# louiskirsch/speechT

Measured on AMD Instinct MI355X. Metric: utterances/sec (training step, 10 s@16 kHz, batch 32), higher is better.
Workload: dtype f32

## Files before the change

include/speecht_hip.h:

```cpp
#ifndef SPEECHT_HIP_H
#define SPEECHT_HIP_H

#include <stddef.h>
#include <stdint.h>

#ifdef __cplusplus
extern "C" {
#endif

#define ST_OK 0
#define ST_EINVAL (-1)
#define ST_ELAUNCH (-2)
#define ST_EWORKSPACE (-3)
#define ST_ECOMM (-4)

typedef struct st_tensor3 {
  float* base;
  int32_t batch;
  int32_t frames;
  int32_t channels;
  int32_t halo;
  int32_t t_pitch;
  int32_t c_pitch;
} st_tensor3;
// ... 21 lines not shown
size_t st_conv1d_fwd_ws(const st_tensor3* x, const st_tensor3* y, int width);
int st_conv1d_nwc_fwd_ws_f32(const st_tensor3* x, const float* packed, const float* bias, int width,
                             int stride, int pad_left, int relu, const st_tensor3* y, void* workspace,
                             size_t workspace_bytes, void* stream);

int st_conv1d_fft_plan(int width, int frames, int batch, int* n, int* valid, int* blocks, int* bins, int* rows_pad);
int st_gemm_nn_batched_f32(const float* a, int64_t lda, int64_t a_batch, const float* b, int64_t b_batch, float* c,
                           int64_t ldc, int64_t c_batch, int m, int k, int n, int batches, void* stream);
size_t st_gemm_nn_batched_ws_bytes(void);
size_t st_gemm_nn_batched_ctrl_bytes(void);
int st_streamk_lost_ptr(void** device_word);
int st_streamk_lost_count(unsigned* count);
int st_streamk_lost_fetch_async(unsigned* host_word, void* stream);
int st_gemm_nn_batched_ws_f32(const float* a, int64_t lda, int64_t a_batch, const float* b, int64_t b_batch, float* c,
                              int64_t ldc, int64_t c_batch, int m, int k, int n, int batches, void* workspace,
                              size_t workspace_bytes, void* stream);
int st_gemm_nn_batched_bt_ws_f32(const float* a, int64_t lda, int64_t a_batch, const float* bt, int64_t bt_batch, float* c,
                                 int64_t ldc, int64_t c_batch, int m, int k, int n, int batches, void* workspace,
                                 size_t workspace_bytes, void* stream);
int st_gemm_tn_batched_f32(const float* a, int64_t lda, int64_t a_batch, const float* z, int64_t ldz, int64_t z_batch,
                           float* out, int64_t out_batch, int m, int k, int n, int batches, void* stream);
int st_gemm_tn_batched_shared_f32(const float* a, int64_t lda, int64_t a_batch, const float* z, int64_t ldz, int64_t z_batch,
                                  float* out, int64_t out_batch, int m, int k, int n, int batches, int z_batch_shift, void* stream);
int st_gemm_nn_g3_batched_f32(const float* a, int64_t lda, int64_t a_batch, const int64_t* a_off, const float* b, int64_t ldb,
                              int64_t b_batch, const int64_t* b_off, int b_transposed, float* c, int64_t ldc, int64_t c_batch,
                              int64_t c_off2, int m, int k, int n, int batches, void* stream);
int st_gemm_tn_g3_batched_f32(const float* a, int64_t lda, int64_t a_batch, const int64_t* a_off, const float* z, int64_t ldz,
                              int64_t z_batch, const int64_t* z_off, float* out, int64_t out_batch, int64_t out_part, int m, int k,
                              int n, int batches, void* stream);
int st_conv1d_fft_three_products(int width, int cin_pitch, int cout);
size_t st_conv1d_fft_table_floats(void);
int st_conv1d_fft_tables_f32(int width, int pad_left, float* tables, size_t table_floats, void* stream);
size_t st_conv1d_fft_filter_floats(int width, int cin_pitch, int cout);
int st_conv1d_fft_filters_f32(const float* packed, int width, int cin, int cout, int cin_pitch, const float* tables, float* gfwd,
                              void* stream);
size_t st_conv1d_fft_sf_floats(const st_tensor3* x, const st_tensor3* y, int width);
size_t st_conv1d_fft_zf_floats(const st_tensor3* dz, int width);
size_t st_conv1d_fft_ws(const st_tensor3* x, const st_tensor3* y, int width);
int st_conv1d_nwc_fwd_fft_f32(const st_tensor3* x, const float* gfwd, const float* bias, int width, int pad_left, int relu,
                              const st_tensor3* y, const float* tables, float* sf, void* workspace,
                              size_t workspace_bytes, void* stream);
int st_conv1d_nwc_fwd_fft_chain_f32(const st_tensor3* x, const float* gfwd, const float* bias, int width, int pad_left, int relu,
                                    const st_tensor3* y, const float* tables, float* sf, int sf_ready, const float* next_tables,
                                    float* next_sf, int next_width, int next_pad_left, int* next_sf_written, void* workspace,
                                    size_t workspace_bytes, void* stream);
int st_conv1d_fft_dz_spectra_f32(const st_tensor3* dz, int width, const float* tables, float* zf, void* stream);
// ... 257 lines not shown
```

speecht_amd/_lib.py:

```python
import ctypes
import os
from ctypes import POINTER, c_char_p, c_float, c_int, c_int32, c_int64, c_long, c_size_t, c_void_p

from .build import LIB_PATH


class Tensor3(ctypes.Structure):
  _fields_ = [('base', c_void_p), ('batch', c_int32), ('frames', c_int32), ('channels', c_int32),
              ('halo', c_int32), ('t_pitch', c_int32), ('c_pitch', c_int32)]


class SpeechtHipError(RuntimeError):
  pass


_T3P = POINTER(Tensor3)
_SIGNATURES = {
    'st_version': (c_int, []),
    'st_last_error': (c_char_p, []),
    'st_trace_begin': (c_int, []),
    'st_trace_begin_timed': (c_int, []),
    'st_trace_timed_filter': (c_int, [c_char_p]),
    'st_trace_end': (c_size_t, [c_char_p, c_size_t]),
    'st_set_tuning': (c_int, [c_char_p, c_int]),
# ... 3 lines not shown
    'st_unpack_filters_f32': (c_int, [c_void_p, c_int, c_int, c_int, c_int, c_void_p, c_void_p]),
    'st_filters_flip_transpose_f32': (c_int, [c_void_p, c_int, c_int, c_int, c_int, c_int, c_void_p, c_void_p]),
    'st_conv1d_nwc_fwd_f32': (c_int, [_T3P, c_void_p, c_void_p, c_int, c_int, c_int, c_int, _T3P, c_void_p]),
    'st_conv1d_fwd_ws': (c_size_t, [_T3P, _T3P, c_int]),
    'st_conv1d_nwc_fwd_ws_f32': (c_int, [_T3P, c_void_p, c_void_p, c_int, c_int, c_int, c_int, _T3P, c_void_p, c_size_t,
                                          c_void_p]),
    'st_conv1d_fft_plan': (c_int, [c_int, c_int, c_int, POINTER(c_int), POINTER(c_int), POINTER(c_int), POINTER(c_int),
                                   POINTER(c_int)]),
    'st_gemm_nn_batched_f32': (c_int, [c_void_p, c_int64, c_int64, c_void_p, c_int64, c_void_p, c_int64, c_int64, c_int, c_int,
                                       c_int, c_int, c_void_p]),
    'st_gemm_nn_batched_ws_bytes': (c_size_t, []),
    'st_gemm_nn_batched_ctrl_bytes': (c_size_t, []),
    'st_streamk_lost_ptr': (c_int, [POINTER(c_void_p)]),
    'st_streamk_lost_count': (c_int, [POINTER(ctypes.c_uint32)]),
    'st_streamk_lost_fetch_async': (c_int, [c_void_p, c_void_p]),
    'st_gemm_nn_batched_ws_f32': (c_int, [c_void_p, c_int64, c_int64, c_void_p, c_int64, c_void_p, c_int64, c_int64, c_int, c_int,
                                          c_int, c_int, c_void_p, c_size_t, c_void_p]),
    'st_gemm_nn_batched_bt_ws_f32': (c_int, [c_void_p, c_int64, c_int64, c_void_p, c_int64, c_void_p, c_int64, c_int64, c_int, c_int,
                                             c_int, c_int, c_void_p, c_size_t, c_void_p]),
    'st_gemm_tn_batched_f32': (c_int, [c_void_p, c_int64, c_int64, c_void_p, c_int64, c_int64, c_void_p, c_int64, c_int, c_int,
                                       c_int, c_int, c_void_p]),
    'st_gemm_tn_batched_shared_f32': (c_int, [c_void_p, c_int64, c_int64, c_void_p, c_int64, c_int64, c_void_p, c_int64, c_int, c_int,
                                              c_int, c_int, c_int, c_void_p]),
    'st_gemm_nn_g3_batched_f32': (c_int, [c_void_p, c_int64, c_int64, POINTER(c_int64), c_void_p, c_int64, c_int64, POINTER(c_int64), c_int,
                                          c_void_p, c_int64, c_int64, c_int64, c_int, c_int, c_int, c_int, c_void_p]),
    'st_gemm_tn_g3_batched_f32': (c_int, [c_void_p, c_int64, c_int64, POINTER(c_int64), c_void_p, c_int64, c_int64, POINTER(c_int64),
                                          c_void_p, c_int64, c_int64, c_int, c_int, c_int, c_int, c_void_p]),
    'st_conv1d_fft_three_products': (c_int, [c_int, c_int, c_int]),
    'st_conv1d_fft_table_floats': (c_size_t, []),
    'st_conv1d_fft_tables_f32': (c_int, [c_int, c_int, c_void_p, c_size_t, c_void_p]),
    'st_conv1d_fft_filter_floats': (c_size_t, [c_int, c_int, c_int]),
    'st_conv1d_fft_filters_f32': (c_int, [c_void_p, c_int, c_int, c_int, c_int, c_void_p, c_void_p, c_void_p]),
    'st_conv1d_fft_sf_floats': (c_size_t, [_T3P, _T3P, c_int]),
    'st_conv1d_fft_zf_floats': (c_size_t, [_T3P, c_int]),
    'st_conv1d_fft_ws': (c_size_t, [_T3P, _T3P, c_int]),
    'st_conv1d_nwc_fwd_fft_f32': (c_int, [_T3P, c_void_p, c_void_p, c_int, c_int, c_int, _T3P, c_void_p, c_void_p, c_void_p,
                                          c_size_t, c_void_p]),
    'st_conv1d_nwc_fwd_fft_chain_f32': (c_int, [_T3P, c_void_p, c_void_p, c_int, c_int, c_int, _T3P, c_void_p, c_void_p, c_int, c_void_p,
                                                c_void_p, c_int, c_int, POINTER(c_int), c_void_p, c_size_t, c_void_p]),
    'st_conv1d_nwc_bwd_data_fft_chain_f32': (c_int, [_T3P, c_void_p, c_void_p, c_int, c_int, _T3P, _T3P, c_void_p, c_void_p, c_void_p, c_int,
                                                     POINTER(c_int), c_void_p, c_size_t, c_void_p]),
    'st_conv1d_fft_filter_plane_elems': (c_size_t, [c_int, c_int, c_int]),
    'st_conv1d_fft_filters_planes': (c_int, [c_void_p, c_int, c_int, c_int, c_int, c_void_p, c_void_p, c_void_p, c_int, c_void_p]),
    'st_conv1d_fft_planes_ws': (c_size_t, [_T3P, _T3P, c_int, c_int]),
    'st_conv1d_nwc_fwd_fft_planes': (c_int, [_T3P, c_void_p, c_void_p, c_void_p, c_int, c_int, c_int, _T3P, c_void_p, c_void_p, c_void_p,
                                             c_int, c_void_p, c_size_t, c_void_p]),
# ... 225 lines not shown
```

speecht_amd/csrc/conv_fft.hip:

```cpp
#include <algorithm>

#include "st_common.h"

namespace {

typedef float f32x2 __attribute__((ext_vector_type(2)));
typedef float f32x4 __attribute__((ext_vector_type(4)));
typedef float f32x16 __attribute__((ext_vector_type(16)));

constexpr int V = 64;
constexpr int KP = 96;
constexpr int HB = KP / 2;
constexpr int T_FS = 0;
constexpr int T_FZ = T_FS + KP * KP;
constexpr int T_IY = T_FZ + KP * KP;
constexpr int T_IX = T_IY + V * KP;
constexpr int T_TW = T_IX + 3 * V * KP;
constexpr int T_FW = T_TW + 256;
constexpr int T_FP = T_FW + HB * 34 * 2;
constexpr int FUSE_BLOCKS = 8, FUSE_HALO = 4, FUSE_Q = 32 + FUSE_HALO;
constexpr int T_IW = T_FP + FUSE_Q * KP * 2;
constexpr int T_ZP = T_IW + KP * KP;
constexpr int T_END = T_ZP + 32 * KP * 2;
__host__ __device__ inline int fused_column(int q, int hh, int n, int pad_left) {
// ... 456 lines not shown
    for (int i = 0; i < 3; ++i)
#pragma unroll
      for (int r = 0; r < 16; ++r) {
        const int m = i * 32 + (r & 3) + 8 * (r >> 2) + 4 * h;
        const int bin = m < HB ? m : m - HB, col = (m < HB ? 0 : half_next) + c;
        if (bin < bins_next) {
          const long o = (long)bin * bin_stride + (long)row * 2 * half_next;
          out[o + col] = sacc[i][r];
          if (out2) out2[o + (m < HB ? half_next : 0) + c] = m < HB ? -sacc[i][r] : sacc[i][r];
        }
      }
  }
}

template <int HP>
__global__ __launch_bounds__(64 * FUSE_BLOCKS, 1) void idft_ola_dft_rows_kernel(
    const float* __restrict__ in, const float* __restrict__ winv, int blocks, int rows_pad, int bins, int half_in, int nchunks, RowsOut y,
    int pad_left, int right, const float* __restrict__ mask, long mask_batch_stride, int mask_c_pitch,
    const float* __restrict__ wz_below, int bins_below, int half_below, float* __restrict__ zf_below) {
  constexpr int NST = 2 * HP / CH;
  static_assert(2 * HP % CH == 0 && HP <= HB / 2, "pairs per term must fill whole stages");
  __shared__ __attribute__((aligned(16))) float wl[KP * KP];
  __shared__ __attribute__((aligned(16))) float wf[32 * KP * 2];
  __shared__ float spill[FUSE_BLOCKS][2][FUSE_HALO][32];
  const int tid = threadIdx.x, lane = tid & 63, l31 = lane & 31, h = lane >> 5;
  const int wave = __builtin_amdgcn_readfirstlane(tid >> 6);
  const int b = blockIdx.x / nchunks, chunk = blockIdx.x - b * nchunks;
  const int j = wave, row = b * blocks + j, c = chunk * 32 + l31;
  const bool active = j < blocks;
  const long plane = (long)rows_pad * 2 * half_in;
  const bool cok = c < half_in;
  const float* src = in + (long)(active ? row : 0) * 2 * half_in + min(c, half_in - 1);
  auto load = [&](float (&bf)[CH], int st) {
#pragma unroll
    for (int s = 0; s < CH; ++s) {
      const int p = st * CH + s;
      const int bin = (p < HP ? 2 * p : 2 * (p - HP)) + h;
      bf[s] = src[(long)min(bin, bins - 1) * plane + (p < HP ? 0 : half_in)];
    }
  };
  float bfr[NST][CH];
  float mk[2][16];
  if (active) {
#pragma unroll
    for (int st = 0; st < NST; ++st) load(bfr[st], st);
    if (mask) {
      const float* mp = mask + (long)b * mask_batch_stride + min(c, mask_c_pitch - 1);
// ... 13 lines not shown
  f32x16 acc[3];
#pragma unroll
  for (int i = 0; i < 3; ++i)
#pragma unroll
    for (int r = 0; r < 16; ++r) acc[i][r] = 0.f;
  if (active) {
    const float* afrag = wl + 2 * l31 + h;
#pragma unroll
    for (int st = 0; st < NST; ++st) {
      __builtin_amdgcn_sched_barrier(0);
#pragma unroll
      for (int s = 0; s < CH; ++s) {
        const int p = st * CH + s;
        const int bin = (p < HP ? 2 * p : 2 * (p - HP)) + h;
        const unsigned keep = (cok && bin < bins) ? 0xffffffffu : 0u;
        const float v = __uint_as_float(__float_as_uint(bfr[st][s]) & keep);
        const int sidx = p < HP ? p : HB / 2 + (p - HP);
#pragma unroll
        for (int i = 0; i < 3; ++i) acc[i] = __builtin_amdgcn_mfma_f32_32x32x2f32(afrag[(sidx * KP + i * 32) * 2], v, acc[i], 0, 0, 0);
      }
      __builtin_amdgcn_sched_barrier(0);
    }
#pragma unroll
    for (int e = 0; e < FUSE_HALO; ++e) spill[j][h][e][l31] = acc[2][e];
  }
  __syncthreads();
  if (!active) return;
#pragma unroll
  for (int e = 0; e < FUSE_HALO; ++e) {
    if (h == 0) { if (j > 0 && e < right) acc[0][e] += spill[j - 1][1][e][l31]; }
    else { if (j + 1 < blocks && e >= FUSE_HALO - pad_left) acc[1][12 + e] += spill[j + 1][0][e - (FUSE_HALO - pad_left)][l31]; }
  }
#pragma unroll
  for (int i = 0; i < 2; ++i)
#pragma unroll
    for (int r = 0; r < 16; ++r) {
      const int t = j * V + i * 32 + (r & 3) + 8 * (r >> 2) + 4 * h;
      float val = c < y.channels ? acc[i][r] : 0.f;
      if (mask) val = mk[i][r] > 0.f ? val : 0.f;
      val = t < y.frames ? val : 0.f;
      asm volatile("" : "+v"(val));
      acc[i][r] = val;
    }
  if (c < y.c_pitch) {
    float* yp = y.base + (long)b * y.batch_stride + c;
#pragma unroll
    for (int i = 0; i < 2; ++i)
#pragma unroll
      for (int r = 0; r < 16; ++r) {
        const int t = j * V + i * 32 + (r & 3) + 8 * (r >> 2) + 4 * h;
        if (t < y.frames) yp[(long)t * y.c_pitch] = acc[i][r];
      }
  }
  if (!wz_below) return;
// ... 359 lines not shown
int st_gemm_nn_batched_ws_f32(const float* a, int64_t lda, int64_t a_batch, const float* b, int64_t b_batch, float* c, int64_t ldc,
                              int64_t c_batch, int m, int k, int n, int batches, void* workspace, size_t workspace_bytes,
                              void* stream) {
  float* sk = (workspace && workspace_bytes >= st_gemm_nn_batched_ws_bytes()) ? reinterpret_cast<float*>(workspace) : nullptr;
  return st::gemm_nn_batched(a, lda, a_batch, b, b_batch, c, ldc, c_batch, m, k, n, batches, st::as_stream(stream), sk);
}

int st_gemm_nn_batched_bt_ws_f32(const float* a, int64_t lda, int64_t a_batch, const float* bt, int64_t bt_batch, float* c, int64_t ldc,
                                 int64_t c_batch, int m, int k, int n, int batches, void* workspace, size_t workspace_bytes,
                                 void* stream) {
  float* sk = (workspace && workspace_bytes >= st_gemm_nn_batched_ws_bytes()) ? reinterpret_cast<float*>(workspace) : nullptr;
  return st::gemm_nn_batched(a, lda, a_batch, bt, bt_batch, c, ldc, c_batch, m, k, n, batches, st::as_stream(stream), sk, true);
}

int st_gemm_tn_batched_f32(const float* a, int64_t lda, int64_t a_batch, const float* z, int64_t ldz, int64_t z_batch, float* out,
                           int64_t out_batch, int m, int k, int n, int batches, void* stream) {
  return st::gemm_tn_batched(a, lda, a_batch, z, ldz, z_batch, out, out_batch, m, k, n, batches, st::as_stream(stream));
}

int st_gemm_tn_batched_shared_f32(const float* a, int64_t lda, int64_t a_batch, const float* z, int64_t ldz, int64_t z_batch, float* out,
                                  int64_t out_batch, int m, int k, int n, int batches, int z_batch_shift, void* stream) {
  ST_REQUIRE(z_batch_shift >= 0 && z_batch_shift < 8, "gemm_tn_batched_shared: bad shift");
  return st::gemm_tn_batched(a, lda, a_batch, z, ldz, z_batch, out, out_batch, m, k, n, batches, st::as_stream(stream), z_batch_shift);
}

int st_gemm_nn_g3_batched_f32(const float* a, int64_t lda, int64_t a_batch, const int64_t* a_off, const float* b, int64_t ldb, int64_t b_batch,
                              const int64_t* b_off, int b_transposed, float* c, int64_t ldc, int64_t c_batch, int64_t c_off2, int m, int k, int n,
                              int batches, void* stream) {
  ST_REQUIRE(a_off && b_off, "gemm_nn_g3_batched: null offsets");
  const long ao[3] = {(long)a_off[0], (long)a_off[1], (long)a_off[2]}, bo[3] = {(long)b_off[0], (long)b_off[1], (long)b_off[2]};
  return st::gemm_nn_g3_batched(a, lda, a_batch, ao, b, ldb, b_batch, bo, c, ldc, c_batch, c_off2, m, k, n, batches, st::as_stream(stream),
                                b_transposed != 0);
}

int st_gemm_tn_g3_batched_f32(const float* a, int64_t lda, int64_t a_batch, const int64_t* a_off, const float* z, int64_t ldz, int64_t z_batch,
                              const int64_t* z_off, float* out, int64_t out_batch, int64_t out_part, int m, int k, int n, int batches,
                              void* stream) {
  ST_REQUIRE(a_off && z_off, "gemm_tn_g3_batched: null offsets");
  const long ao[3] = {(long)a_off[0], (long)a_off[1], (long)a_off[2]}, zo[3] = {(long)z_off[0], (long)z_off[1], (long)z_off[2]};
  return st::gemm_tn_g3_batched(a, lda, a_batch, ao, z, ldz, z_batch, zo, out, out_batch, out_part, m, k, n, batches, st::as_stream(stream));
}

int st_conv1d_fft_three_products(int width, int cin_pitch, int cout) {
  return g3_form(width, cin_pitch, cout) ? 2 : (zf3_form(width, cout) ? 1 : 0);
}

// ... 398 lines not shown
```

speecht_amd/csrc/conv_gemm.hip:

```cpp
#include <algorithm>
#include <atomic>
#include <cmath>
#include <cstdlib>

#include <type_traits>

#include "st_common.h"
#include "streamk_map.h"

namespace {

typedef float f32x16 __attribute__((ext_vector_type(16)));
typedef float f32x4 __attribute__((ext_vector_type(4)));

constexpr int BK = 32;
constexpr int APITCH = BK + 4;
constexpr int NTHREADS = 256;

struct RowMap {
  int frames;
  int row_stride;
  long batch_stride;
  long row0;
  __device__ __forceinline__ long off(int m) const {
// ... 7 lines not shown
  const float* A;  RowMap amap;
  const float* Bm; int Np;
  float* C;        RowMap cmap;
  const float* mask; RowMap mmap;
  const float* bias;
  int M, Kvalid, Kp, n_store, relu;
  int taps, cp;
  int tiles_m, tiles_n, chunk;
  int gm, tm_per, tn_per;
  int splits, steps_per_split;
  float* slab;
  float* colsum;
  int colsum_rows;
  int batches;
  long a_batch, b_batch, c_batch;
  long bt_ld; int bt_rows;
};


__device__ __forceinline__ void dma16_sv(unsigned lds_byte_addr, const void* sbase, unsigned voff_bytes) {
  unsigned keep;
  asm volatile("s_mov_b32 %0, m0\n\ts_mov_b32 m0, %1\n\ts_nop 0\n\tglobal_load_lds_dwordx4 %2, %3\n\ts_mov_b32 m0, %0"
               : "=&s"(keep) : "s"(lds_byte_addr), "v"(voff_bytes), "s"(sbase) : "memory");
}
__device__ __forceinline__ void dma_wait_all() { asm volatile("s_waitcnt vmcnt(0)" ::: "memory"); }
__device__ __forceinline__ unsigned lds_addr(const float* p) {
  return (unsigned)(size_t)(__attribute__((address_space(3))) const float*)p;
}

template <int N> struct FVec;
template <> struct FVec<1> { typedef float type; };
template <> struct FVec<2> { typedef float type __attribute__((ext_vector_type(2))); };
template <> struct FVec<4> { typedef float type __attribute__((ext_vector_type(4))); };
template <int N> __device__ __forceinline__ float vget(const typename FVec<N>::type& v, int i) { return v[i]; }
template <> __device__ __forceinline__ float vget<1>(const float& v, int) { return v; }
template <int N> __device__ __forceinline__ void vset(typename FVec<N>::type& v, int i, float x) { v[i] = x; }
template <> __device__ __forceinline__ void vset<1>(float& v, int, float x) { v = x; }

__device__ __forceinline__ int swz_slot4(int lane, int row) { return ((lane & 7) ^ ((row >> 1) & 7)) * 4; }
__device__ __forceinline__ int swz_frag(int row, int q, int h) { return row * BK + (((2 * q + h) ^ ((row >> 1) & 7)) * 4); }

template <int BM, int BN, int WMW, int WNW, bool BT>
struct NNStage {
  static constexpr int WTM = BM / WMW, WTN = BN / WNW;
  static constexpr int MT = WTM / 32, NT = WTN / 32;
  static constexpr int A_DMA = BM / 32;
// ... 346 lines not shown
    }
  }
  if (EPI == 1 && p.colsum) {
    bvec out;
#pragma unroll
    for (int n = 0; n < NT; ++n) vset<NT>(out, n, csum[n] + __shfl_xor(csum[n], 32, 64));
    if (h == 0) *reinterpret_cast<bvec*>(p.colsum + (long)(tile_m * WMW + wm) * p.Np + col0) = out;
  }
}

__device__ unsigned g_sk_lost = 0;

struct BinsParams {
  const float* A; const float* B; float* C;
  long lda, ldb, ldc, a_batch, b_batch, c_batch;
  int tiles_m, tiles_n;
  st::SkPlan plan;
  unsigned* ctrl;
  float* partial;
  unsigned epoch;
  unsigned pub_epoch;
};

template <int BM, int BN, int WMW, int WNW, int MINW, bool BT>
__global__ __launch_bounds__(NTHREADS, MINW) void gemm_nn_bins_kernel(BinsParams p) {
  typedef NNStage<BM, BN, WMW, WNW, BT> S;
  constexpr int WTM = S::WTM, WTN = S::WTN, MT = S::MT, NT = S::NT;
  constexpr int A_DMA = S::A_DMA, B_DMA = S::B_DMA, N_DMA = S::N_DMA, A_SZ = S::A_SZ, B_SZ = S::B_SZ;
  constexpr int B_LPR = BN / 4;
  static_assert(WMW * WNW == 4 && MT >= 1 && NT == 2 && A_DMA >= 1 && B_DMA >= 1, "tile config");
  typedef typename FVec<NT>::type bvec;
  typedef unsigned long long u64;

  __shared__ __attribute__((aligned(16))) float smem[2 * A_SZ + 2 * B_SZ + 4];
  float* const As = smem;
  float* const Bs = smem + 2 * A_SZ;
  volatile int* const sk_lost_p = reinterpret_cast<volatile int*>(smem + 2 * A_SZ + 2 * B_SZ);

  const int tid = threadIdx.x;
  const int lane = tid & 63;
  const int wave = __builtin_amdgcn_readfirstlane(tid >> 6);
  const int l31 = lane & 31, h = lane >> 5;
  const int wm = wave / WNW, wn = wave % WNW;
  if (tid == 0) *sk_lost_p = 0;

  const int xcd = blockIdx.x & 7, local = blockIdx.x >> 3;
  const int slot = blockIdx.x;
  st::SkCursor cur;
  if (!st::sk_begin(p.plan, xcd, local, cur)) return;
  const int per_bin = p.tiles_m * p.tiles_n;

  int a_lane[A_DMA];
#pragma unroll
  for (int i = 0; i < A_DMA; ++i) {
    const int row = (wave * A_DMA + i) * 8 + (lane >> 3);
    a_lane[i] = row * (int)p.lda + swz_slot4(lane, row);
  }
  int b_lane[B_DMA];
#pragma unroll
  for (int i = 0; i < B_DMA; ++i) {
    if (BT) {
      const int row = (wave * B_DMA + i) * 8 + (lane >> 3);
      b_lane[i] = row * (int)p.ldb + swz_slot4(lane, row);
    } else {
      b_lane[i] = ((wave * B_DMA + i) * (64 / B_LPR) + lane / B_LPR) * (int)p.ldb + (lane % B_LPR) * 4;
    }
  }
  int bt_frag[4];
  {
    const int row = wn * WTN + l31;
#pragma unroll
    for (int q = 0; q < 4; ++q) bt_frag[q] = swz_frag(row, q, h);
  }
  int a_frag[4];
  {
    const int row = wm * WTM + l31;
#pragma unroll
    for (int q = 0; q < 4; ++q) a_frag[q] = swz_frag(row, q, h);
  }
  const int b_frag = (4 * h) * BN + wn * WTN + NT * l31;
  const int tcol = wn * WTN + NT * l31;

  while (cur.u < cur.u_end) {
    const st::SkPiece pc = st::sk_piece(p.plan, cur);
    cur.u += pc.kt1 - pc.kt0;
    const int bin = pc.tile / per_bin, t = pc.tile - bin * per_bin;
    const int tile_n = t / p.tiles_m, tile_m = t - tile_n * p.tiles_m;
    const int m0 = tile_m * BM, n0 = tile_n * BN;
    const float* __restrict__ Ab = p.A + (long)bin * p.a_batch + (long)m0 * p.lda;
    const float* __restrict__ Bb = p.B + (long)bin * p.b_batch + (BT ? (long)n0 * p.ldb : (long)n0);
    const float* aptr[A_DMA];
    const float* bptr[B_DMA];
#pragma unroll
    for (int i = 0; i < A_DMA; ++i) aptr[i] = Ab + a_lane[i];
#pragma unroll
    for (int i = 0; i < B_DMA; ++i) bptr[i] = Bb + b_lane[i];
    auto dma_piece = [&](int pcx, int k0, int buf) {
      if (pcx < A_DMA) {
        const int i = pcx < A_DMA ? pcx : 0;
        __builtin_amdgcn_global_load_lds((st::gptr_t)(aptr[i] + k0), (st::lptr_t)(As + buf * A_SZ + (wave * A_DMA + i) * 256), 16, 0, 0);
      } else {
        const int i = pcx - A_DMA < B_DMA ? pcx - A_DMA : 0;
        __builtin_amdgcn_global_load_lds((st::gptr_t)(BT ? bptr[i] + k0 : bptr[i] + (long)k0 * p.ldb), (st::lptr_t)(Bs + buf * B_SZ + (wave * B_DMA + i) * 256), 16, 0, 0);
      }
    };

    f32x16 acc[MT][NT] = {};

    int k0 = pc.kt0 * BK;
#pragma unroll
    for (int pcx = 0; pcx < N_DMA; ++pcx) dma_piece(pcx, k0, 0);
    __syncthreads();

    auto stage = [&](auto cur_c, auto more_c) {
      const int nk0 = k0 + BK;
      k0 = nk0;
      S::template run<decltype(cur_c)::value, decltype(more_c)::value>(As, Bs, a_frag, bt_frag, b_frag, acc, 4, dma_piece, nk0);
    };
    const int nk = pc.kt1 - pc.kt0;
    nn_stage_pairs(nk, stage);

    if (pc.kt0 > 0) {
      float* const mine = p.partial + (long)slot * (BM * BN);
#pragma unroll
      for (int i = 0; i < MT; ++i)
#pragma unroll
        for (int r = 0; r < 16; ++r) {
          const int row = wm * WTM + i * 32 + (r & 3) + 8 * (r >> 2) + 4 * h;
          const u64 bits = (u64)__float_as_uint(acc[i][0][r]) | ((u64)__float_as_uint(acc[i][1][r]) << 32);
          __hip_atomic_store(reinterpret_cast<u64*>(mine + row * BN + tcol), bits, __ATOMIC_RELAXED, __HIP_MEMORY_SCOPE_AGENT);
        }
      asm volatile("s_waitcnt vmcnt(0)" ::: "memory");
      __syncthreads();
      if (tid == 0) __hip_atomic_store(p.ctrl + st::SK_FLAGS + slot, p.pub_epoch, __ATOMIC_RELAXED, __HIP_MEMORY_SCOPE_AGENT);
      continue;
    }
    int covered = pc.kt1, src = slot;
    while (covered < p.plan.nk) {
      src += 8;
      if (tid == 0) {
        unsigned* flag = p.ctrl + st::SK_FLAGS + src;
        unsigned spins = 0;
        while (__hip_atomic_load(flag, __ATOMIC_RELAXED, __HIP_MEMORY_SCOPE_AGENT) != p.epoch) {
          __builtin_amdgcn_s_sleep(8);
          if (++spins > (1u << 21)) {
            __hip_atomic_fetch_add(p.ctrl + st::SK_TIMEOUTS, 1u, __ATOMIC_RELAXED, __HIP_MEMORY_SCOPE_AGENT);
            __hip_atomic_fetch_add(&g_sk_lost, 1u, __ATOMIC_RELAXED, __HIP_MEMORY_SCOPE_AGENT);
            *sk_lost_p = 1;
            break;
          }
        }
        __hip_atomic_store(flag, 0u, __ATOMIC_RELAXED, __HIP_MEMORY_SCOPE_AGENT);
      }
      __syncthreads();
      const float poison = *sk_lost_p ? __uint_as_float(0x7fc00000u) : 0.f;
      const float* const theirs = p.partial + (long)src * (BM * BN);
#pragma unroll
      for (int i = 0; i < MT; ++i) {
        u64 part[16];
#pragma unroll
        for (int r = 0; r < 16; ++r) {
          const int row = wm * WTM + i * 32 + (r & 3) + 8 * (r >> 2) + 4 * h;
          part[r] = __hip_atomic_load(reinterpret_cast<const u64*>(theirs + row * BN + tcol), __ATOMIC_RELAXED, __HIP_MEMORY_SCOPE_AGENT);
        }
#pragma unroll
        for (int r = 0; r < 16; ++r) {
          acc[i][0][r] += __uint_as_float((unsigned)part[r]) + poison;
          acc[i][1][r] += __uint_as_float((unsigned)(part[r] >> 32)) + poison;
        }
      }
      covered += min(p.plan.upw, p.plan.nk - covered);
    }
    float* __restrict__ Cb = p.C + (long)bin * p.c_batch + (long)m0 * p.ldc + n0 + (BT ? wn * WTN + l31 : tcol);
#pragma unroll
    for (int i = 0; i < MT; ++i)
#pragma unroll
      for (int r = 0; r < 16; ++r) {
        const int row = wm * WTM + i * 32 + (r & 3) + 8 * (r >> 2) + 4 * h;
        if (BT) {
#pragma unroll
          for (int n = 0; n < NT; ++n) Cb[(long)row * p.ldc + n * 32] = acc[i][n][r];
        } else {
          bvec out;
#pragma unroll
          for (int n = 0; n < NT; ++n) vset<NT>(out, n, acc[i][n][r]);
          *reinterpret_cast<bvec*>(Cb + (long)row * p.ldc) = out;
        }
      }
  }
}

struct G3Params {
  const float* A; long lda, a_batch; long a_off[3];
  const float* B; long ldb, b_batch; long b_off[3];
  float* C; long ldc, c_batch, c_off2;
  int M, K, N;
  int tiles_m, tiles_n, batches, ksplit;
};

__global__ __launch_bounds__(256) void g3_zero_out_kernel(float* __restrict__ C, long ldc, long c_batch, long c_off2, int M, int N) {
  const int m = blockIdx.x * 4 + (threadIdx.x >> 6);
  if (m >= M) return;
  float* row = C + (long)blockIdx.y * c_batch + (long)m * ldc;
  for (int c = (threadIdx.x & 63) * 4; c < N; c += 256) {
    *reinterpret_cast<f32x4*>(row + c) = f32x4{0.f, 0.f, 0.f, 0.f};
    *reinterpret_cast<f32x4*>(row + c_off2 + c) = f32x4{0.f, 0.f, 0.f, 0.f};
  }
}

// ... 688 lines not shown
      launch_nn<128, 128, 2, 2, true>(p, epi, s);
    else if (tiles128 >= 192 || p.splits > 1) launch_nn<128, 128, 2, 2>(p, epi, s);
    else launch_nn<64, 128, 2, 2>(p, epi, s);
  } else if (p.Np == 64) {
    launch_nn<128, 64, 2, 2>(p, epi, s);
  } else if (p.Np == 32) {
    launch_nn<128, 32, 4, 1>(p, epi, s);
  } else {
    st::set_error("unsupported packed width n_pad=%d", p.Np);
    return ST_EINVAL;
  }
  return st::check_launch("gemm_nn");
}

}

int st::gemm_nn_batched(const float* A, long lda, long a_batch, const float* B, long b_batch, float* C, long ldc,
                        long c_batch, int M, int K, int N, int batches, hipStream_t s, float* sk_ws, bool b_transposed) {
  if (!(A && B && C && M > 0 && K > 0 && K % 32 == 0 && N % 128 == 0 && batches > 0 && lda % 4 == 0 && ldc % 4 == 0)) {
    st::set_error("gemm_nn_batched: bad shape M=%d K=%d N=%d", M, K, N);
    return ST_EINVAL;
  }
  const int knob = st::tuning(st::TUNE_STREAMK);
  if (sk_ws && knob != 2 && M % 64 == 0 && a_batch % 4 == 0 && b_batch % 4 == 0 && (long)64 * lda < (1L << 30) && (long)32 * N < (1L << 30)) {
    const long tiles = (long)batches * (M / 64) * (N / 128);
    const double per_cu = (double)tiles / 256.0;
    const bool uneven = tiles > 256 && tiles <= 768 && std::ceil(per_cu) / per_cu > 1.2;
    int slots = st::tuning(st::TUNE_STREAMK_SLOTS);
    if (slots != 64 && slots != 96) slots = 64;
    st::SkPlan plan;
    if ((knob == 1 || uneven) && tiles < (1L << 24) && st::sk_make_plan((int)tiles, K / BK, slots, plan)) {
      static std::atomic<unsigned> g_epoch{0};
      unsigned epoch = g_epoch.fetch_add(1, std::memory_order_relaxed) + 1;
      if (epoch == 0) epoch = g_epoch.fetch_add(1, std::memory_order_relaxed) + 1;
      BinsParams q{};
      q.A = A; q.B = B; q.C = C;
      q.lda = lda; q.ldb = b_transposed ? K : N; q.ldc = ldc;
      q.a_batch = a_batch; q.b_batch = b_batch; q.c_batch = c_batch;
      q.tiles_m = M / 64; q.tiles_n = N / 128;
      q.plan = plan;
      q.ctrl = reinterpret_cast<unsigned*>(sk_ws);
      q.partial = sk_ws + st::SK_CTRL_WORDS;
      q.epoch = epoch;
      q.pub_epoch = st::tuning(st::TUNE_STREAMK_TEST_DROP) ? (epoch ^ 0x80000000u) : epoch;
      st::trace("gemm_nn_bins<64,128,2,2%s> batched bins=%d M=%d Np=%d Kp=%d streamk wgs=%d upw=%d gflop=%.3f", b_transposed ? ",bt" : "",
                batches, M, N, K, 8 * plan.wgs_per_xcd, plan.upw, 2e-9 * M * (double)N * K * batches);
      {
        st::LaunchTimer timer(s);
        const dim3 grid(8 * plan.wgs_per_xcd), block(NTHREADS);
        if (b_transposed) {
          if (plan.wgs_per_xcd > 64) st::launch_timed(timer, gemm_nn_bins_kernel<64, 128, 2, 2, 3, true>, grid, block, s, q);
          else st::launch_timed(timer, gemm_nn_bins_kernel<64, 128, 2, 2, 2, true>, grid, block, s, q);
        } else {
          if (plan.wgs_per_xcd > 64) st::launch_timed(timer, gemm_nn_bins_kernel<64, 128, 2, 2, 3, false>, grid, block, s, q);
          else st::launch_timed(timer, gemm_nn_bins_kernel<64, 128, 2, 2, 2, false>, grid, block, s, q);
        }
      }
      return st::check_launch("gemm_nn_bins");
    }
  }
  if (M % 128 == 64 && M > 128 && (long)K * N >= (1L << 21) && (long)st::ceil_div(M, 128) * (N / 128) * batches >= 512) {
    if (int e = st::gemm_nn_batched(A, lda, a_batch, B, b_batch, C, ldc, c_batch, M - 64, K, N, batches, s, nullptr, b_transposed)) return e;
    return st::gemm_nn_batched(A + (long)(M - 64) * lda, lda, a_batch, B, b_batch, C + (long)(M - 64) * ldc, ldc, c_batch, 64, K, N, batches, s,
                               nullptr, b_transposed);
  }
  NNParams p{};
  p.A = A;
  p.amap.frames = M; p.amap.row_stride = (int)lda; p.amap.batch_stride = 0; p.amap.row0 = 0;
  p.Bm = B;
  p.Np = N;
  p.C = C;
  p.cmap.frames = M; p.cmap.row_stride = (int)ldc; p.cmap.batch_stride = 0; p.cmap.row0 = 0;
  p.M = M;
  p.Kvalid = K;
  p.Kp = K;
  p.n_store = N;
  p.taps = 1;
  p.cp = K;
  p.batches = batches;
  p.a_batch = a_batch; p.b_batch = b_batch; p.c_batch = c_batch;
  if (b_transposed) { p.bt_ld = K; p.bt_rows = N; }
  return run_nn(p, 0, s);
}

int st::gemm_tn_batched(const float* A, long lda, long a_batch, const float* Z, long ldz, long z_batch, float* out,
                        long o_batch, int M, int K, int N, int batches, hipStream_t s, int z_batch_shift) {
  if (!(A && Z && out && M > 0 && M % 32 == 0 && K % 128 == 0 && N % 128 == 0 && batches > 0)) {
    st::set_error("gemm_tn_batched: bad shape M=%d K=%d N=%d", M, K, N);
    return ST_EINVAL;
  }
  TNParams p{};
  p.A = A;
  p.amap.frames = M; p.amap.row_stride = (int)lda; p.amap.batch_stride = 0; p.amap.row0 = 0;
  p.Z = Z;
  p.zmap.frames = M; p.zmap.row_stride = (int)ldz; p.zmap.batch_stride = 0; p.zmap.row0 = 0;
  p.M = M;
  p.Kvalid = K;
  p.Kp = K;
  p.Np = N;
  p.z_cols = N;
  p.rows_per_split = M;
  p.out = out;
  p.tiles_k = K / 128;
  p.tiles_n = N / 128;
  p.amap_batches = 1;
  p.adv_b = 32 / M;
  p.adv_t = 32 % M;
  p.a_batch = a_batch; p.z_batch = z_batch; p.o_batch = o_batch;
  p.z_shift = z_batch_shift;
  st::trace("gemm_tn<128> batched bins=%d M=%d Kp=%d Np=%d gflop=%.3f", batches, M, K, N, 2e-9 * M * (double)K * N * batches);
  {
    st::LaunchTimer timer(s);
    st::launch_timed(timer, gemm_tn_kernel<128, 2, 2>, dim3(p.tiles_k * p.tiles_n, 1, batches), dim3(TN_THREADS), s, p);
  }
  return st::check_launch("gemm_tn_batched");
}

int st::gemm_nn_g3_batched(const float* A, long lda, long a_batch, const long a_off[3], const float* B, long ldb, long b_batch,
                           const long b_off[3], float* C, long ldc, long c_batch, long c_off2, int M, int K, int N, int batches,
                           hipStream_t s, bool b_transposed) {
  if (!(A && B && C && M > 0 && K > 0 && K % 64 == 0 && N % 128 == 0 && batches > 0 && lda % 4 == 0 && ldb % 4 == 0 && ldc % 4 == 0 &&
        c_off2 % 4 == 0 && a_off[0] % 4 == 0 && a_off[1] % 4 == 0 && a_off[2] % 4 == 0 && b_off[0] % 4 == 0 && b_off[1] % 4 == 0 && b_off[2] % 4 == 0)) {
    st::set_error("gemm_nn_g3_batched: bad shape M=%d K=%d N=%d", M, K, N);
    return ST_EINVAL;
  }
  if (M % 128 == 64 && M > 128 && (long)batches * st::ceil_div(M, 128) * (N / 128) >= 512 &&
      st::tuning(st::TUNE_G3_TILE) == 0) {
    if (int e = st::gemm_nn_g3_batched(A, lda, a_batch, a_off, B, ldb, b_batch, b_off, C, ldc, c_batch, c_off2, M - 64, K, N, batches, s, b_transposed)) return e;
    return st::gemm_nn_g3_batched(A + (long)(M - 64) * lda, lda, a_batch, a_off, B, ldb, b_batch, b_off, C + (long)(M - 64) * ldc, ldc, c_batch, c_off2,
                                  64, K, N, batches, s, b_transposed);
  }
  G3Params p{};
  p.A = A; p.lda = lda; p.a_batch = a_batch;
  p.B = B; p.ldb = ldb; p.b_batch = b_batch;
  for (int i = 0; i < 3; ++i) { p.a_off[i] = a_off[i]; p.b_off[i] = b_off[i]; }
  p.C = C; p.ldc = ldc; p.c_batch = c_batch; p.c_off2 = c_off2;
// ... 411 lines not shown
```

speecht_amd/csrc/st_common.h:

```cpp
#pragma once
#include <hip/hip_runtime.h>
#include <hip/hip_ext.h>
#include <stdarg.h>
#include <stdio.h>

#include "speecht_hip.h"

namespace st {

void set_error(const char* fmt, ...);

bool trace_on();
void trace(const char* fmt, ...);
class LaunchTimer {
 public:
  explicit LaunchTimer(hipStream_t s);
  bool active() const { return start_ != nullptr; }
  hipEvent_t start() const { return start_; }
  hipEvent_t stop() const { return stop_; }

 private:
  hipEvent_t start_, stop_;
};
template <typename... KArgs, typename... Args>
inline void launch_timed(const LaunchTimer& t, void (*kernel)(KArgs...), const dim3& grid, const dim3& block, hipStream_t s,
                         Args&&... args) {
  static_assert(sizeof...(KArgs) == sizeof...(Args), "launch_timed: argument count does not match the kernel");
  if (t.active()) hipExtLaunchKernelGGL(kernel, grid, block, 0, s, t.start(), t.stop(), 0, static_cast<KArgs>(args)...);
  else hipLaunchKernelGGL(kernel, grid, block, 0, s, static_cast<KArgs>(args)...);
}
enum { TUNE_STREAMK, TUNE_STREAMK_SLOTS, TUNE_STREAMK_TEST_DROP, TUNE_NO_FUSED_TRANSFORMS, TUNE_BF16_LAG_COPIES, TUNE_FILTERS_IDFT_VALU,
       TUNE_BF16_TAPS_PANEL, TUNE_NO_G3, TUNE_G3_TILE, TUNE_COUNT };
int tuning(int key);

constexpr int SK_FLAGS = 0, SK_TIMEOUTS = 768, SK_CTRL_WORDS = 1024;
constexpr long SK_WS_FLOATS = SK_CTRL_WORDS + 768L * 64 * 128;
int gemm_nn_batched(const float* A, long lda, long a_batch, const float* B, long b_batch, float* C, long ldc, long c_batch,
                    int M, int K, int N, int batches, hipStream_t s, float* sk_ws = nullptr, bool b_transposed = false);
int gemm_tn_batched(const float* A, long lda, long a_batch, const float* Z, long ldz, long z_batch, float* out, long o_batch,
                    int M, int K, int N, int batches, hipStream_t s, int z_batch_shift = 0);
int gemm_nn_g3_batched(const float* A, long lda, long a_batch, const long a_off[3], const float* B, long ldb, long b_batch,
                       const long b_off[3], float* C, long ldc, long c_batch, long c_off2, int M, int K, int N, int batches,
                       hipStream_t s, bool b_transposed = false);
int gemm_tn_g3_batched(const float* A, long lda, long a_batch, const long a_off[3], const float* Z, long ldz, long z_batch,
                       const long z_off[3], float* out, long o_batch, long o_part, int M, int K, int N, int batches, hipStream_t s);

int gemm_bf16_bins(int planes, const void* a_planes, size_t a_plane, long a_rows_apart, long a_bin, const void* bt_planes,
                   size_t b_plane, long ldb, long b_bin, float* c, long ldc, int rows, int k, int n, int bins, hipStream_t s,
                   int b_bin_shift = 0);
int lag_products_tr_bf16(const void* s_plane, const void* z_plane, int bins, int rows, int half, int npo, float* q, hipStream_t s);
bool conv_taps_bf16_eligible(const st_tensor3& a, const st_tensor3& y, int width, int lead, const st_tensor3* act);
int conv_taps_bf16(const st_tensor3& a, const void* a_plane, const void* filters, const float* bias, int width, int lead, int relu,
                   const st_tensor3* act, const void* act_plane, const st_tensor3& y, void* y_plane, hipStream_t s);
int transpose_bf16_bins(const void* src, void* dst, int bins, int rows, int cols, hipStream_t s);
int transpose_bf16_bins_split(const void* src, void* dst, int bins, int rows, int cols, int forms, hipStream_t s);

inline hipStream_t as_stream(void* s) { return reinterpret_cast<hipStream_t>(s); }

inline int check_launch(const char* what) {
  hipError_t e = hipGetLastError();
  if (e != hipSuccess) {
    set_error("%s: %s", what, hipGetErrorString(e));
    return ST_ELAUNCH;
// ... 42 lines not shown
```

Baseline: 4868.

## Add 64-wide TN gemm tile, reuse LDS for spill, byte-offset addressing in bins gemm

The TN gemm gains a 64-column tile variant, chosen automatically when the 128-wide tiling would leave a partial second wave on the GPU. The fused FFT conv kernel keeps its halo spill buffer in unused parts of the wl shared array instead of a separate allocation, which reduces LDS use. The stream-K bins gemm switches to precomputed unsigned byte offsets to save address registers and arithmetic, and is now fixed at 3 waves per SIMD in its launch bounds. This adds extra guards on ldc/K ranges, and the tile heuristic may pick a less efficient tile for some shapes.

```diff
diff --git a/include/speecht_hip.h b/include/speecht_hip.h
--- a/include/speecht_hip.h
+++ b/include/speecht_hip.h
@@ -67,6 +67,9 @@
                            float* out, int64_t out_batch, int m, int k, int n, int batches, void* stream);
 int st_gemm_tn_batched_shared_f32(const float* a, int64_t lda, int64_t a_batch, const float* z, int64_t ldz, int64_t z_batch,
                                   float* out, int64_t out_batch, int m, int k, int n, int batches, int z_batch_shift, void* stream);
+int st_gemm_tn_batched_tile_f32(const float* a, int64_t lda, int64_t a_batch, const float* z, int64_t ldz, int64_t z_batch,
+                                float* out, int64_t out_batch, int m, int k, int n, int batches, int z_batch_shift, int tile_n,
+                                void* stream);
 int st_gemm_nn_g3_batched_f32(const float* a, int64_t lda, int64_t a_batch, const int64_t* a_off, const float* b, int64_t ldb,
                               int64_t b_batch, const int64_t* b_off, int b_transposed, float* c, int64_t ldc, int64_t c_batch,
                               int64_t c_off2, int m, int k, int n, int batches, void* stream);
diff --git a/speecht_amd/_lib.py b/speecht_amd/_lib.py
--- a/speecht_amd/_lib.py
+++ b/speecht_amd/_lib.py
@@ -49,6 +49,8 @@
                                        c_int, c_int, c_void_p]),
     'st_gemm_tn_batched_shared_f32': (c_int, [c_void_p, c_int64, c_int64, c_void_p, c_int64, c_int64, c_void_p, c_int64, c_int, c_int,
                                               c_int, c_int, c_int, c_void_p]),
+    'st_gemm_tn_batched_tile_f32': (c_int, [c_void_p, c_int64, c_int64, c_void_p, c_int64, c_int64, c_void_p, c_int64, c_int, c_int,
+                                            c_int, c_int, c_int, c_int, c_void_p]),
     'st_gemm_nn_g3_batched_f32': (c_int, [c_void_p, c_int64, c_int64, POINTER(c_int64), c_void_p, c_int64, c_int64, POINTER(c_int64), c_int,
                                           c_void_p, c_int64, c_int64, c_int64, c_int, c_int, c_int, c_int, c_void_p]),
     'st_gemm_tn_g3_batched_f32': (c_int, [c_void_p, c_int64, c_int64, POINTER(c_int64), c_void_p, c_int64, c_int64, POINTER(c_int64),
diff --git a/speecht_amd/csrc/conv_fft.hip b/speecht_amd/csrc/conv_fft.hip
--- a/speecht_amd/csrc/conv_fft.hip
+++ b/speecht_amd/csrc/conv_fft.hip
@@ -502,7 +502,11 @@
   static_assert(2 * HP % CH == 0 && HP <= HB / 2, "pairs per term must fill whole stages");
   __shared__ __attribute__((aligned(16))) float wl[KP * KP];
   __shared__ __attribute__((aligned(16))) float wf[32 * KP * 2];
-  __shared__ float spill[FUSE_BLOCKS][2][FUSE_HALO][32];
+  constexpr int SPILL = FUSE_BLOCKS * FUSE_HALO * 32;
+  constexpr bool SPILL_IN_WL = (HB / 2 - HP) * KP * 2 >= SPILL;
+  __shared__ float spill_own[SPILL_IN_WL ? 32 : 2 * SPILL];
+  float* const spill_before = SPILL_IN_WL ? wl + HP * KP * 2 : spill_own;
+  float* const spill_after = SPILL_IN_WL ? wl + (HB / 2 + HP) * KP * 2 : spill_own + SPILL;
   const int tid = threadIdx.x, lane = tid & 63, l31 = lane & 31, h = lane >> 5;
   const int wave = __builtin_amdgcn_readfirstlane(tid >> 6);
   const int b = blockIdx.x / nchunks, chunk = blockIdx.x - b * nchunks;
@@ -562,14 +566,14 @@
       __builtin_amdgcn_sched_barrier(0);
     }
 #pragma unroll
-    for (int e = 0; e < FUSE_HALO; ++e) spill[j][h][e][l31] = acc[2][e];
+    for (int e = 0; e < FUSE_HALO; ++e) (h ? spill_after : spill_before)[(j * FUSE_HALO + e) * 32 + l31] = acc[2][e];
   }
   __syncthreads();
   if (!active) return;
 #pragma unroll
   for (int e = 0; e < FUSE_HALO; ++e) {
-    if (h == 0) { if (j > 0 && e < right) acc[0][e] += spill[j - 1][1][e][l31]; }
-    else { if (j + 1 < blocks && e >= FUSE_HALO - pad_left) acc[1][12 + e] += spill[j + 1][0][e - (FUSE_HALO - pad_left)][l31]; }
+    if (h == 0) { if (j > 0 && e < right) acc[0][e] += spill_after[((j - 1) * FUSE_HALO + e) * 32 + l31]; }
+    else { if (j + 1 < blocks && e >= FUSE_HALO - pad_left) acc[1][12 + e] += spill_before[((j + 1) * FUSE_HALO + e - (FUSE_HALO - pad_left)) * 32 + l31]; }
   }
 #pragma unroll
   for (int i = 0; i < 2; ++i)
@@ -975,6 +979,13 @@
                                   int64_t out_batch, int m, int k, int n, int batches, int z_batch_shift, void* stream) {
   ST_REQUIRE(z_batch_shift >= 0 && z_batch_shift < 8, "gemm_tn_batched_shared: bad shift");
   return st::gemm_tn_batched(a, lda, a_batch, z, ldz, z_batch, out, out_batch, m, k, n, batches, st::as_stream(stream), z_batch_shift);
+}
+
+int st_gemm_tn_batched_tile_f32(const float* a, int64_t lda, int64_t a_batch, const float* z, int64_t ldz, int64_t z_batch, float* out,
+                                int64_t out_batch, int m, int k, int n, int batches, int z_batch_shift, int tile_n, void* stream) {
+  ST_REQUIRE(z_batch_shift >= 0 && z_batch_shift < 8, "gemm_tn_batched_tile: bad shift");
+  ST_REQUIRE(tile_n == 64 || tile_n == 128, "gemm_tn_batched_tile: tile_n is 64 or 128");
+  return st::gemm_tn_batched(a, lda, a_batch, z, ldz, z_batch, out, out_batch, m, k, n, batches, st::as_stream(stream), z_batch_shift, tile_n);
 }
 
 int st_gemm_nn_g3_batched_f32(const float* a, int64_t lda, int64_t a_batch, const int64_t* a_off, const float* b, int64_t ldb, int64_t b_batch,
diff --git a/speecht_amd/csrc/conv_gemm.hip b/speecht_amd/csrc/conv_gemm.hip
--- a/speecht_amd/csrc/conv_gemm.hip
+++ b/speecht_amd/csrc/conv_gemm.hip
@@ -53,6 +53,12 @@
   unsigned keep;
   asm volatile("s_mov_b32 %0, m0\n\ts_mov_b32 m0, %1\n\ts_nop 0\n\tglobal_load_lds_dwordx4 %2, %3\n\ts_mov_b32 m0, %0"
                : "=&s"(keep) : "s"(lds_byte_addr), "v"(voff_bytes), "s"(sbase) : "memory");
+}
+__device__ __forceinline__ float* at_bytes(float* ubase, unsigned voff_bytes) {
+  return reinterpret_cast<float*>(reinterpret_cast<char*>(ubase) + voff_bytes);
+}
+__device__ __forceinline__ const float* at_bytes(const float* ubase, unsigned voff_bytes) {
+  return reinterpret_cast<const float*>(reinterpret_cast<const char*>(ubase) + voff_bytes);
 }
 __device__ __forceinline__ void dma_wait_all() { asm volatile("s_waitcnt vmcnt(0)" ::: "memory"); }
 __device__ __forceinline__ unsigned lds_addr(const float* p) {
@@ -445,8 +451,8 @@
   unsigned pub_epoch;
 };
 
-template <int BM, int BN, int WMW, int WNW, int MINW, bool BT>
-__global__ __launch_bounds__(NTHREADS, MINW) void gemm_nn_bins_kernel(BinsParams p) {
+template <int BM, int BN, int WMW, int WNW, bool BT>
+__global__ __launch_bounds__(NTHREADS, 3) void gemm_nn_bins_kernel(BinsParams p) {
   typedef NNStage<BM, BN, WMW, WNW, BT> S;
   constexpr int WTM = S::WTM, WTN = S::WTN, MT = S::MT, NT = S::NT;
   constexpr int A_DMA = S::A_DMA, B_DMA = S::B_DMA, N_DMA = S::N_DMA, A_SZ = S::A_SZ, B_SZ = S::B_SZ;
@@ -473,20 +479,20 @@
   if (!st::sk_begin(p.plan, xcd, local, cur)) return;
   const int per_bin = p.tiles_m * p.tiles_n;
 
-  int a_lane[A_DMA];
+  unsigned a_lane[A_DMA];
 #pragma unroll
   for (int i = 0; i < A_DMA; ++i) {
     const int row = (wave * A_DMA + i) * 8 + (lane >> 3);
-    a_lane[i] = row * (int)p.lda + swz_slot4(lane, row);
-  }
-  int b_lane[B_DMA];
+    a_lane[i] = (unsigned)(row * (int)p.lda + swz_slot4(lane, row)) * 4u;
+  }
+  unsigned b_lane[B_DMA];
 #pragma unroll
   for (int i = 0; i < B_DMA; ++i) {
     if (BT) {
       const int row = (wave * B_DMA + i) * 8 + (lane >> 3);
-      b_lane[i] = row * (int)p.ldb + swz_slot4(lane, row);
+      b_lane[i] = (unsigned)(row * (int)p.ldb + swz_slot4(lane, row)) * 4u;
     } else {
-      b_lane[i] = ((wave * B_DMA + i) * (64 / B_LPR) + lane / B_LPR) * (int)p.ldb + (lane % B_LPR) * 4;
+      b_lane[i] = (unsigned)(((wave * B_DMA + i) * (64 / B_LPR) + lane / B_LPR) * (int)p.ldb + (lane % B_LPR) * 4) * 4u;
     }
   }
   int bt_frag[4];
@@ -503,6 +509,10 @@
   }
   const int b_frag = (4 * h) * BN + wn * WTN + NT * l31;
   const int tcol = wn * WTN + NT * l31;
+  const int lrow = wm * WTM + 4 * h;
+  const unsigned part_lane = (unsigned)(lrow * BN + tcol) * 4u;
+  const unsigned c_lane = (unsigned)(lrow * (int)p.ldc + (BT ? wn * WTN + l31 : tcol)) * 4u;
+  auto trow = [](int i, int r) { return i * 32 + (r & 3) + 8 * (r >> 2); };
 
   while (cur.u < cur.u_end) {
     const st::SkPiece pc = st::sk_piece(p.plan, cur);
@@ -512,19 +522,13 @@
     const int m0 = tile_m * BM, n0 = tile_n * BN;
     const float* __restrict__ Ab = p.A + (long)bin * p.a_batch + (long)m0 * p.lda;
     const float* __restrict__ Bb = p.B + (long)bin * p.b_batch + (BT ? (long)n0 * p.ldb : (long)n0);
-    const float* aptr[A_DMA];
-    const float* bptr[B_DMA];
-#pragma unroll
-    for (int i = 0; i < A_DMA; ++i) aptr[i] = Ab + a_lane[i];
-#pragma unroll
-    for (int i = 0; i < B_DMA; ++i) bptr[i] = Bb + b_lane[i];
     auto dma_piece = [&](int pcx, int k0, int buf) {
       if (pcx < A_DMA) {
         const int i = pcx < A_DMA ? pcx : 0;
-        __builtin_amdgcn_global_load_lds((st::gptr_t)(aptr[i] + k0), (st::lptr_t)(As + buf * A_SZ + (wave * A_DMA + i) * 256), 16, 0, 0);
+        __builtin_amdgcn_global_load_lds((st::gptr_t)at_bytes(Ab + k0, a_lane[i]), (st::lptr_t)(As + buf * A_SZ + (wave * A_DMA + i) * 256), 16, 0, 0);
       } else {
         const int i = pcx - A_DMA < B_DMA ? pcx - A_DMA : 0;
-        __builtin_amdgcn_global_load_lds((st::gptr_t)(BT ? bptr[i] + k0 : bptr[i] + (long)k0 * p.ldb), (st::lptr_t)(Bs + buf * B_SZ + (wave * B_DMA + i) * 256), 16, 0, 0);
+        __builtin_amdgcn_global_load_lds((st::gptr_t)at_bytes(BT ? Bb + k0 : Bb + (long)k0 * p.ldb, b_lane[i]), (st::lptr_t)(Bs + buf * B_SZ + (wave * B_DMA + i) * 256), 16, 0, 0);
       }
     };
 
@@ -549,9 +553,8 @@
       for (int i = 0; i < MT; ++i)
 #pragma unroll
         for (int r = 0; r < 16; ++r) {
-          const int row = wm * WTM + i * 32 + (r & 3) + 8 * (r >> 2) + 4 * h;
           const u64 bits = (u64)__float_as_uint(acc[i][0][r]) | ((u64)__float_as_uint(acc[i][1][r]) << 32);
-          __hip_atomic_store(reinterpret_cast<u64*>(mine + row * BN + tcol), bits, __ATOMIC_RELAXED, __HIP_MEMORY_SCOPE_AGENT);
+          __hip_atomic_store(reinterpret_cast<u64*>(at_bytes(mine + trow(i, r) * BN, part_lane)), bits, __ATOMIC_RELAXED, __HIP_MEMORY_SCOPE_AGENT);
         }
       asm volatile("s_waitcnt vmcnt(0)" ::: "memory");
       __syncthreads();
@@ -582,10 +585,8 @@
       for (int i = 0; i < MT; ++i) {
         u64 part[16];
 #pragma unroll
-        for (int r = 0; r < 16; ++r) {
-          const int row = wm * WTM + i * 32 + (r & 3) + 8 * (r >> 2) + 4 * h;
-          part[r] = __hip_atomic_load(reinterpret_cast<const u64*>(theirs + row * BN + tcol), __ATOMIC_RELAXED, __HIP_MEMORY_SCOPE_AGENT);
-        }
+        for (int r = 0; r < 16; ++r)
+          part[r] = __hip_atomic_load(reinterpret_cast<const u64*>(at_bytes(theirs + trow(i, r) * BN, part_lane)), __ATOMIC_RELAXED, __HIP_MEMORY_SCOPE_AGENT);
 #pragma unroll
         for (int r = 0; r < 16; ++r) {
           acc[i][0][r] += __uint_as_float((unsigned)part[r]) + poison;
@@ -594,20 +595,20 @@
       }
       covered += min(p.plan.upw, p.plan.nk - covered);
     }
-    float* __restrict__ Cb = p.C + (long)bin * p.c_batch + (long)m0 * p.ldc + n0 + (BT ? wn * WTN + l31 : tcol);
+    float* __restrict__ Cb = p.C + (long)bin * p.c_batch + (long)m0 * p.ldc + n0;
 #pragma unroll
     for (int i = 0; i < MT; ++i)
 #pragma unroll
       for (int r = 0; r < 16; ++r) {
-        const int row = wm * WTM + i * 32 + (r & 3) + 8 * (r >> 2) + 4 * h;
+        float* const crow = Cb + (long)trow(i, r) * p.ldc;
         if (BT) {
 #pragma unroll
-          for (int n = 0; n < NT; ++n) Cb[(long)row * p.ldc + n * 32] = acc[i][n][r];
+          for (int n = 0; n < NT; ++n) *at_bytes(crow + n * 32, c_lane) = acc[i][n][r];
         } else {
           bvec out;
 #pragma unroll
           for (int n = 0; n < NT; ++n) vset<NT>(out, n, acc[i][n][r]);
-          *reinterpret_cast<bvec*>(Cb + (long)row * p.ldc) = out;
+          *reinterpret_cast<bvec*>(at_bytes(crow, c_lane)) = out;
         }
       }
   }
@@ -1342,7 +1343,8 @@
     return ST_EINVAL;
   }
   const int knob = st::tuning(st::TUNE_STREAMK);
-  if (sk_ws && knob != 2 && M % 64 == 0 && a_batch % 4 == 0 && b_batch % 4 == 0 && (long)64 * lda < (1L << 30) && (long)32 * N < (1L << 30)) {
+  if (sk_ws && knob != 2 && M % 64 == 0 && a_batch % 4 == 0 && b_batch % 4 == 0 && (long)64 * lda < (1L << 30) && (long)32 * N < (1L << 30) &&
+      (long)64 * ldc < (1L << 29) && (!b_transposed || (long)128 * K < (1L << 29))) {
     const long tiles = (long)batches * (M / 64) * (N / 128);
     const double per_cu = (double)tiles / 256.0;
     const bool uneven = tiles > 256 && tiles <= 768 && std::ceil(per_cu) / per_cu > 1.2;
@@ -1368,13 +1370,8 @@
       {
         st::LaunchTimer timer(s);
         const dim3 grid(8 * plan.wgs_per_xcd), block(NTHREADS);
-        if (b_transposed) {
-          if (plan.wgs_per_xcd > 64) st::launch_timed(timer, gemm_nn_bins_kernel<64, 128, 2, 2, 3, true>, grid, block, s, q);
-          else st::launch_timed(timer, gemm_nn_bins_kernel<64, 128, 2, 2, 2, true>, grid, block, s, q);
-        } else {
-          if (plan.wgs_per_xcd > 64) st::launch_timed(timer, gemm_nn_bins_kernel<64, 128, 2, 2, 3, false>, grid, block, s, q);
-          else st::launch_timed(timer, gemm_nn_bins_kernel<64, 128, 2, 2, 2, false>, grid, block, s, q);
-        }
+        if (b_transposed) st::launch_timed(timer, gemm_nn_bins_kernel<64, 128, 2, 2, true>, grid, block, s, q);
+        else st::launch_timed(timer, gemm_nn_bins_kernel<64, 128, 2, 2, false>, grid, block, s, q);
       }
       return st::check_launch("gemm_nn_bins");
     }
@@ -1404,10 +1401,14 @@
 }
 
 int st::gemm_tn_batched(const float* A, long lda, long a_batch, const float* Z, long ldz, long z_batch, float* out,
-                        long o_batch, int M, int K, int N, int batches, hipStream_t s, int z_batch_shift) {
-  if (!(A && Z && out && M > 0 && M % 32 == 0 && K % 128 == 0 && N % 128 == 0 && batches > 0)) {
-    st::set_error("gemm_tn_batched: bad shape M=%d K=%d N=%d", M, K, N);
+                        long o_batch, int M, int K, int N, int batches, hipStream_t s, int z_batch_shift, int tile_n) {
+  if (!(A && Z && out && M > 0 && M % 32 == 0 && K % 128 == 0 && N % 128 == 0 && batches > 0 && (tile_n == 0 || tile_n == 64 || tile_n == 128))) {
+    st::set_error("gemm_tn_batched: bad shape M=%d K=%d N=%d tile_n=%d", M, K, N, tile_n);
     return ST_EINVAL;
+  }
+  if (tile_n == 0) {
+    const long tiles128 = (long)batches * (K / 128) * (N / 128);
+    tile_n = (tiles128 > 256 && tiles128 <= 320 && M <= 512) ? 64 : 128;
   }
   TNParams p{};
   p.A = A;
@@ -1422,16 +1423,18 @@
   p.rows_per_split = M;
   p.out = out;
   p.tiles_k = K / 128;
-  p.tiles_n = N / 128;
+  p.tiles_n = N / tile_n;
   p.amap_batches = 1;
   p.adv_b = 32 / M;
   p.adv_t = 32 % M;
   p.a_batch = a_batch; p.z_batch = z_batch; p.o_batch = o_batch;
   p.z_shift = z_batch_shift;
-  st::trace("gemm_tn<128> batched bins=%d M=%d Kp=%d Np=%d gflop=%.3f", batches, M, K, N, 2e-9 * M * (double)K * N * batches);
+  st::trace("gemm_tn<%d> batched bins=%d M=%d Kp=%d Np=%d gflop=%.3f", tile_n, batches, M, K, N, 2e-9 * M * (double)K * N * batches);
   {
     st::LaunchTimer timer(s);
-    st::launch_timed(timer, gemm_tn_kernel<128, 2, 2>, dim3(p.tiles_k * p.tiles_n, 1, batches), dim3(TN_THREADS), s, p);
+    const dim3 grid(p.tiles_k * p.tiles_n, 1, batches);
+    if (tile_n == 64) st::launch_timed(timer, gemm_tn_kernel<64, 2, 2>, grid, dim3(TN_THREADS), s, p);
+    else st::launch_timed(timer, gemm_tn_kernel<128, 2, 2>, grid, dim3(TN_THREADS), s, p);
   }
   return st::check_launch("gemm_tn_batched");
 }
diff --git a/speecht_amd/csrc/st_common.h b/speecht_amd/csrc/st_common.h
--- a/speecht_amd/csrc/st_common.h
+++ b/speecht_amd/csrc/st_common.h
@@ -38,7 +38,7 @@
 int gemm_nn_batched(const float* A, long lda, long a_batch, const float* B, long b_batch, float* C, long ldc, long c_batch,
                     int M, int K, int N, int batches, hipStream_t s, float* sk_ws = nullptr, bool b_transposed = false);
 int gemm_tn_batched(const float* A, long lda, long a_batch, const float* Z, long ldz, long z_batch, float* out, long o_batch,
-                    int M, int K, int N, int batches, hipStream_t s, int z_batch_shift = 0);
+                    int M, int K, int N, int batches, hipStream_t s, int z_batch_shift = 0, int tile_n = 0);
 int gemm_nn_g3_batched(const float* A, long lda, long a_batch, const long a_off[3], const float* B, long ldb, long b_batch,
                        const long b_off[3], float* C, long ldc, long c_batch, long c_off2, int M, int K, int N, int batches,
                        hipStream_t s, bool b_transposed = false);
```

Result: faster. 4926 (median of 6 runs) (+1.2%).
